# karltan0328/POPE

Hardware: AMD Instinct MI355X
Metric: image-pairs/s (DINOv2-S/14 extract+match, 640x480) (higher is better)
Workload: dtype f16x3 (fp32 operands split hi+lo into f16, 3 MFMAs per product, fp32 accumulate)

## Files before the change

### pope_amd/csrc/gemm_rowln.hip

```cpp
#include "gemm_core.h"
#include "gemm_routes.h"

namespace {

typedef _Float16 f16x4 __attribute__((ext_vector_type(4)));
typedef _Float16 f16x8 __attribute__((ext_vector_type(8)));
typedef __attribute__((ext_vector_type(4))) unsigned u32x4;
typedef __attribute__((ext_vector_type(2))) unsigned u32x2;

constexpr int RN = 384, RK = 32;
constexpr int ROWB = 64;
template <int RM_, int NWM_> struct RlGeo {
    static constexpr int RM = RM_, NWM = NWM_, NW = 4 * NWM, RTH = 64 * NW;
    static constexpr int NMI = RM / NWM / 16;
    static constexpr int STAGE_H = (RM + RN) * ROWB;
    static constexpr size_t STATS_OFF = size_t(2) * STAGE_H * sizeof(_Float16);
    static constexpr size_t CTAB_OFF = STATS_OFF + size_t(2) * 4 * RM * sizeof(float);
    static constexpr size_t PF_OFF = CTAB_OFF + size_t(4) * RN * sizeof(float);
    static constexpr size_t LDS_BYTES = PF_OFF + size_t(NW) * 256;
    static constexpr int EROWS = size_t(NW) * 16 * 100 * sizeof(float) <= size_t(STAGE_H) * sizeof(_Float16) ? 16 : 8;
    static constexpr int AROWS = RM / NW, WROWS = RN / NW;
    static constexpr int NPF = (RM * 12 + RTH - 1) / RTH;
    static_assert(size_t(NW) * EROWS * 100 * sizeof(float) <= size_t(STAGE_H) * sizeof(_Float16), "transposition buffers must fit a stage");
    static_assert(LDS_BYTES <= 160 * 1024, "LDS of a CU");
    static_assert(WROWS % 8 == 0 && AROWS % 8 == 0 && RM == NWM * NMI * 16, "eight rows per staging instruction");
};
typedef __attribute__((address_space(3))) void* lds_void_ptr;
constexpr float A_SCALE = K_PLANES_ACT_SCALE, W_SCALE = K_PLANES_W_SCALE;

__device__ __forceinline__ int pope_lane_id() {
    unsigned z = 0;
    asm volatile("" : "+s"(z));
    return int(__builtin_amdgcn_mbcnt_hi(~0u, __builtin_amdgcn_mbcnt_lo(~0u, z)));
}
__device__ __forceinline__ f32x4 mfma16(f16x8 a, f16x8 b, f32x4 c) {
    return __builtin_amdgcn_mfma_f32_16x16x32_f16(a, b, c, 0, 0, 0);
}
__device__ __forceinline__ float quad_sum(float v) {
    float a, b;
    pope_xor16_pair(v, a, b);
    pope_xor32_pair(a + b, a, b);
    return a + b;
}

#ifdef RL_STAMPS
__device__ unsigned long long g_rl_dbg[3][64];
#define RL_STAMP(slot)                                                                                             \
    do {                                                                                                           \
        if (LN && blockIdx.x == 0 && threadIdx.x == 0 && rl_si + (slot) < 64)        \
            g_rl_dbg[g.K == 384 ? 0 : (g.K == 1536 ? 1 : 2)][rl_si + (slot)] = wall_clock64();                     \
    } while (0)
#else
#define RL_STAMP(slot) do {} while (0)
#endif

__device__ __forceinline__ void rl_barrier() {
    __builtin_amdgcn_fence(__ATOMIC_RELEASE, "workgroup", "local");
    __builtin_amdgcn_s_barrier();
    __builtin_amdgcn_fence(__ATOMIC_ACQUIRE, "workgroup", "local");
}

enum { RL_LN_PLANES = 0, RL_LN_F32 = 1, RL_BIAS_PLANES = 2, RL_GELU_PLANES = 3 };

template <class G, int MODE, bool RES_TABLE>
__global__ __launch_bounds__(G::RTH) void gemm_rowln16_kernel(const GemmParams g, int n_tiles, int ncol) {
    constexpr bool LN = MODE == RL_LN_PLANES || MODE == RL_LN_F32, LN_PLANES = MODE == RL_LN_PLANES;
    constexpr int RM = G::RM, NMI = G::NMI, RTH = G::RTH, STAGE_H = G::STAGE_H, EROWS = G::EROWS, AROWS = G::AROWS, WROWS = G::WROWS;
    constexpr int WMR = 16 * NMI;
    constexpr int NIA = AROWS / 8, NIW = WROWS / 8;
    extern __shared__ __attribute__((aligned(16))) float smem[];
    _Float16* lds = reinterpret_cast<_Float16*>(smem);
    float* stats = reinterpret_cast<float*>(reinterpret_cast<char*>(smem) + G::STATS_OFF);
    float* ctab = reinterpret_cast<float*>(reinterpret_cast<char*>(smem) + G::CTAB_OFF);

    const int tid = threadIdx.x, lane = tid & 63;
    const int wave = __builtin_amdgcn_readfirstlane(tid >> 6);
    const int wm = wave >> 2, wn = wave & 3;
    const int nk = g.K / RK;
    const unsigned lda4 = unsigned(g.lda) * 4u, ldw4 = unsigned(g.ldw) * 4u;
    const __amdgpu_buffer_rsrc_t ra = __builtin_amdgcn_make_buffer_rsrc(const_cast<void*>(g.a_pl), 0, unsigned(g.M) * lda4, 0x00020000);
    const __amdgpu_buffer_rsrc_t rw = __builtin_amdgcn_make_buffer_rsrc(const_cast<void*>(g.w_pl), 0, unsigned(g.N) * ldw4, 0x00020000);
    auto row_tile = [&](int t) -> int { return LN ? t : t / ncol; };
    auto col_tile = [&](int t) -> int { return LN ? 0 : t - (t / ncol) * ncol; };

    const int grid = gridDim.x, full_rounds = n_tiles / grid;
    const int remapped = xcd_remap(blockIdx.x, grid);
    const int tail_cand = full_rounds * grid + int(blockIdx.x);
    const int tail_tile = tail_cand < n_tiles ? tail_cand : n_tiles;
    auto tile_of = [&](int ord) -> int {
        const int in_tail = pope_uniform_select(ord == full_rounds, tail_tile, n_tiles);
        return pope_uniform_select(ord < full_rounds, ord * grid + remapped, in_tail);
    };
    const int first = tile_of(0);
    if (first >= n_tiles) return;
    if (LN && tid < RN) {
        const float gm = g.gamma ? g.gamma[tid] : 1.0f;
        ctab[tid] = gm * (1.0f / (A_SCALE * W_SCALE));
        ctab[RN + tid] = (g.bias ? g.bias[tid] : 0.f) * gm;
        ctab[2 * RN + tid] = g.ln_w[tid];
        ctab[3 * RN + tid] = g.ln_b[tid];
    }

    const unsigned a8 = 8u * lda4, w8 = 8u * ldw4;
    auto dma = [&](int stage, int t, int kt_) {
        int ln_ = pope_lane_id();
        asm volatile("" : "+v"(ln_));
        const int r8 = ln_ >> 3, piece = (ln_ & 7) ^ r8;
        const int lt = t < n_tiles ? t : n_tiles - 1;
        _Float16* S_ = lds + stage * STAGE_H;
        const unsigned vt = unsigned(row_tile(lt) * RM + AROWS * wave + r8) * lda4 + unsigned(piece) * 16u;
        const unsigned ko = unsigned(kt_) * 128u + unsigned(col_tile(lt)) * unsigned(RN) * ldw4;
        const unsigned vw0 = unsigned(WROWS * wave + r8) * ldw4 + unsigned(piece) * 16u;
#pragma unroll
        for (int i = 0; i < NIA; ++i)
            __builtin_amdgcn_raw_ptr_buffer_load_lds(ra, (lds_void_ptr)(S_ + (AROWS * wave + 8 * i) * ROWB), 16, vt + i * a8, unsigned(kt_) * 128u, 0, LN ? 3 : 0);
#pragma unroll
        for (int i = 0; i < NIW; ++i)
            __builtin_amdgcn_raw_ptr_buffer_load_lds(rw, (lds_void_ptr)(S_ + (RM + WROWS * wave + 8 * i) * ROWB), 16, vw0, ko + i * w8, 0, 0);
    };
    f32x4 acc[NMI][6];
    auto zero_acc = [&]() {
#pragma unroll
        for (int mi = 0; mi < NMI; ++mi)
#pragma unroll
            for (int ni = 0; ni < 6; ++ni) acc[mi][ni] = f32x4{0.f, 0.f, 0.f, 0.f};
    };

    const __amdgpu_buffer_rsrc_t rx = __builtin_amdgcn_make_buffer_rsrc(g.C, 0, unsigned(g.M) * unsigned(RN) * 4u, 0x00020000);
    const __amdgpu_buffer_rsrc_t rln = __builtin_amdgcn_make_buffer_rsrc(LN_PLANES ? g.ln_planes : static_cast<void*>(g.ln_f32), 0,
                                                                         unsigned(g.M) * unsigned(RN) * 4u, 0x00020000);
    const __amdgpu_buffer_rsrc_t rres = __builtin_amdgcn_make_buffer_rsrc(
        const_cast<float*>(g.res), 0, unsigned(RES_TABLE ? g.res_mod : g.M) * unsigned(g.ldres) * 4u, 0x00020000);

    lds_void_ptr pf_pad = (lds_void_ptr)(reinterpret_cast<char*>(smem) + G::PF_OFF + wave * 256);
    auto prefetch_res = [&](int tile_, int j) {
        int t_ = wave * 64 + pope_lane_id();
        asm volatile("" : "+v"(t_));
        const unsigned L = unsigned(t_) + unsigned(RTH) * unsigned(j), row = L / 12u, pc = L - 12u * row;
        const unsigned off = RM * 12 % RTH == 0 || L < unsigned(RM * 12) ? (unsigned(tile_) * RM + row) * unsigned(RN) * 4u + pc * 128u : 0xFFFFFF00u;
        __builtin_amdgcn_raw_ptr_buffer_load_lds(rres, pf_pad, 4, off, 0, 0, 0);
    };

    int rl_si = 0;
    [[maybe_unused]] auto epilogue = [&](int tile, int free_stage) {
        const int m0 = tile * RM;
        float* wreg = reinterpret_cast<float*>(lds + free_stage * STAGE_H) + wave * (EROWS * 100);
        int elane = pope_lane_id();
        asm volatile("" : "+v"(elane));
        RL_STAMP(1);
        int l15 = elane & 15, q4 = elane >> 4;
        asm volatile("" : "+v"(l15), "+v"(q4));
        const int er = l15 & (EROWS - 1);
#pragma unroll
        for (int mi = 0; mi < NMI; ++mi)
#pragma unroll
            for (int ni = 0; ni < 6; ++ni) asm volatile("" : "+v"(acc[mi][ni]));
        const int col0 = wn * 96 + 4 * q4;
#pragma unroll
        for (int ni = 0; ni < 6; ++ni) {
            const f32x4 gam = *reinterpret_cast<const f32x4*>(ctab + col0 + 16 * ni);
            const f32x4 bia = *reinterpret_cast<const f32x4*>(ctab + RN + col0 + 16 * ni);
#pragma unroll
            for (int mi = 0; mi < NMI; ++mi) {
                const unsigned row = unsigned(m0 + wm * WMR + mi * 16 + l15);
                const unsigned rr = RES_TABLE ? row % unsigned(g.res_mod) : row;
                const f32x4 r = __builtin_bit_cast(f32x4, __builtin_amdgcn_raw_buffer_load_b128(
                                    rres, rr * unsigned(g.ldres) * 4u + unsigned(col0) * 4u, ni * 64, 0));
                acc[mi][ni] = r + acc[mi][ni] * gam + bia;
            }
#pragma unroll
            for (int mi = 0; mi < NMI; ++mi) asm volatile("" : "+v"(acc[mi][ni]));
            __builtin_amdgcn_sched_barrier(0);
        }
        __builtin_amdgcn_sched_barrier(0);
        RL_STAMP(2);
        const int rl = wm * WMR + l15;
#pragma unroll
        for (int mi = 0; mi < NMI; ++mi) {
            float s = 0.f;
#pragma unroll
            for (int ni = 0; ni < 6; ++ni) s += (acc[mi][ni][0] + acc[mi][ni][1]) + (acc[mi][ni][2] + acc[mi][ni][3]);
            s = quad_sum(s);
            if (q4 == 0) stats[wn * RM + rl + 16 * mi] = s;
        }
        rl_barrier();
        float mean[NMI], rstd[NMI];
#pragma unroll
        for (int mi = 0; mi < NMI; ++mi) {
            const float* p = stats + rl + 16 * mi;
            mean[mi] = ((p[0] + p[RM]) + (p[2 * RM] + p[3 * RM])) * (1.0f / float(RN));
        }
        __builtin_amdgcn_sched_barrier(0);
        RL_STAMP(3);
        auto store_lines = [&](const __amdgpu_buffer_rsrc_t& rdst, int row_base) {
            int el = elane;
            asm volatile("" : "+v"(el));
            const int epiece = el & 7;
#pragma unroll
            for (int t = 0; t < (EROWS * 3) / 8; ++t) {
                const int L = t * 8 + (el >> 3), row = (L * 43) >> 7, ln = L - 3 * row;
                const f32x4 v = *reinterpret_cast<const f32x4*>(&wreg[row * 100 + ln * 32 + epiece * 4]);
                const unsigned off = unsigned(row_base + row) * unsigned(RN) * 4u + unsigned(wn * 96 + ln * 32 + epiece * 4) * 4u;
                __builtin_amdgcn_raw_buffer_store_b128(__builtin_bit_cast(u32x4, v), rdst, off, 0, 0);
            }
        };
#pragma unroll
        for (int mi = 0; mi < NMI; ++mi) {
#pragma unroll
            for (int h = 0; h < 16 / EROWS; ++h) {
                if (EROWS == 16 || (l15 >> 3) == h) {
#pragma unroll
                    for (int ni = 0; ni < 6; ++ni) *reinterpret_cast<f32x4*>(&wreg[er * 100 + ni * 16 + 4 * q4]) = acc[mi][ni];
                }
                __builtin_amdgcn_wave_barrier();
                store_lines(rx, m0 + wm * WMR + mi * 16 + h * EROWS);
                __builtin_amdgcn_wave_barrier();
            }
        }
#pragma unroll
        for (int mi = 0; mi < NMI; ++mi) {
            float qs = 0.f;
#pragma unroll
            for (int ni = 0; ni < 6; ++ni) {
                const f32x4 d = acc[mi][ni] - mean[mi];
                acc[mi][ni] = d;
                qs += (d[0] * d[0] + d[1] * d[1]) + (d[2] * d[2] + d[3] * d[3]);
            }
            qs = quad_sum(qs);
            if (q4 == 0) stats[4 * RM + wn * RM + rl + 16 * mi] = qs;
        }
        rl_barrier();
#pragma unroll
        for (int mi = 0; mi < NMI; ++mi) {
            const float* p = stats + 4 * RM + rl + 16 * mi;
            const float var = ((p[0] + p[RM]) + (p[2 * RM] + p[3 * RM])) * (1.0f / float(RN));
            rstd[mi] = 1.0f / sqrtf(var + g.ln_eps);
        }
        __builtin_amdgcn_sched_barrier(0);
        RL_STAMP(4);
        const int live = g.M - (m0 + rl);
        float finite_probe = 0.f;
#pragma unroll
        for (int mi = 0; mi < NMI; ++mi) finite_probe += 16 * mi < live ? __builtin_fabsf(mean[mi]) + rstd[mi] : 0.f;
        f32x2 amax = {0.f, 0.f};
#pragma unroll
        for (int mi = 0; mi < NMI; ++mi) {
#pragma unroll
            for (int h = 0; h < 16 / EROWS; ++h) {
                if (EROWS == 16 || (l15 >> 3) == h) {
#pragma unroll
                    for (int ni = 0; ni < 6; ++ni) {
                        const f32x4 lw = *reinterpret_cast<const f32x4*>(ctab + 2 * RN + col0 + 16 * ni);
                        const f32x4 lb = *reinterpret_cast<const f32x4*>(ctab + 3 * RN + col0 + 16 * ni);
                        const f32x4 y = acc[mi][ni] * rstd[mi] * lw + lb;
                        if constexpr (LN_PLANES) {
                            const f32x4 ys = y * A_SCALE;
                            pope_amax4x2(amax, 16 * mi < live ? ys : f32x4{0.f, 0.f, 0.f, 0.f});
                            f16x4 hi, lo;
                            pope_split4(ys, hi, lo);
                            const int c = ni * 16 + 4 * q4;
                            _Float16* hp = reinterpret_cast<_Float16*>(wreg) + er * 200 + pope_planes_col(c);
                            *reinterpret_cast<f16x4*>(hp) = hi;
                            *reinterpret_cast<f16x4*>(hp + 32) = lo;
                        } else {
                            *reinterpret_cast<f32x4*>(&wreg[er * 100 + ni * 16 + 4 * q4]) = y;
                        }
                    }
                }
                __builtin_amdgcn_wave_barrier();
                store_lines(rln, m0 + wm * WMR + mi * 16 + h * EROWS);
                __builtin_amdgcn_wave_barrier();
            }
        }
        if constexpr (LN_PLANES)
            pope_range_flag(g.range_flag, POPE_RANGE_LAYERNORM,
                            !(__builtin_fmaxf(amax[0], amax[1]) < POPE_F16_OVERFLOW) ||
                                !(finite_probe < INFINITY));
        RL_STAMP(5);
    };

    const __amdgpu_buffer_rsrc_t rcp = __builtin_amdgcn_make_buffer_rsrc(LN ? static_cast<void*>(g.C) : g.c_pl, 0,
                                                                         unsigned(g.M) * unsigned(g.ldc) * 4u, 0x00020000);
    [[maybe_unused]] auto epilogue_planes = [&](int tile, int free_stage) {
        const int m0 = row_tile(tile) * RM, n0 = col_tile(tile) * RN;
        float* wreg = reinterpret_cast<float*>(lds + free_stage * STAGE_H) + wave * (EROWS * 100);
        int elane = pope_lane_id();
        asm volatile("" : "+v"(elane));
        int l15 = elane & 15, q4 = elane >> 4;
        asm volatile("" : "+v"(l15), "+v"(q4));
        const int er = l15 & (EROWS - 1);
#pragma unroll
        for (int mi = 0; mi < NMI; ++mi)
#pragma unroll
            for (int ni = 0; ni < 6; ++ni) asm volatile("" : "+v"(acc[mi][ni]));
        const int col0 = n0 + wn * 96 + 4 * q4;
        constexpr float inv = 1.0f / (A_SCALE * W_SCALE);
        f32x4 bias[6];
#pragma unroll
        for (int ni = 0; ni < 6; ++ni) bias[ni] = g.bias ? *reinterpret_cast<const f32x4*>(g.bias + col0 + 16 * ni) : f32x4{0.f, 0.f, 0.f, 0.f};
        f32x2 amax = {0.f, 0.f};
#pragma unroll
        for (int mi = 0; mi < NMI; ++mi) {
#pragma unroll
            for (int h = 0; h < 16 / EROWS; ++h) {
                if (EROWS == 16 || (l15 >> 3) == h) {
#pragma unroll
                    for (int ni = 0; ni < 6; ++ni) {
                        f32x4 v = acc[mi][ni] * inv + bias[ni];
                        if constexpr (MODE == RL_GELU_PLANES) {
                            const f32x2 g01 = pope_gelu_erf_pair(f32x2{v[0], v[1]}), g23 = pope_gelu_erf_pair(f32x2{v[2], v[3]});
                            v = f32x4{g01[0], g01[1], g23[0], g23[1]};
                        }
                        pope_amax4x2(amax, v);
                        f16x4 hi, lo;
                        pope_split4(v * A_SCALE, hi, lo);
                        const int c = ni * 16 + 4 * q4;
                        _Float16* hp = reinterpret_cast<_Float16*>(wreg) + er * 200 + pope_planes_col(c);
                        *reinterpret_cast<f16x4*>(hp) = hi;
                        *reinterpret_cast<f16x4*>(hp + 32) = lo;
                    }
                }
                __builtin_amdgcn_wave_barrier();
                {
                    int el = elane;
                    asm volatile("" : "+v"(el));
                    const int epiece = el & 7;
                    const int row_base = m0 + wm * WMR + mi * 16 + h * EROWS;
#pragma unroll
                    for (int t = 0; t < (EROWS * 3) / 8; ++t) {
                        const int L = t * 8 + (el >> 3), row = (L * 43) >> 7, ln = L - 3 * row;
                        const f32x4 v = *reinterpret_cast<const f32x4*>(&wreg[row * 100 + ln * 32 + epiece * 4]);
                        const unsigned off = unsigned(row_base + row) * unsigned(g.ldc) * 4u + unsigned(n0 + wn * 96 + ln * 32 + epiece * 4) * 4u;
                        __builtin_amdgcn_raw_buffer_store_b128(__builtin_bit_cast(u32x4, v), rcp, off, 0, 2);
                    }
                }
                __builtin_amdgcn_wave_barrier();
            }
        }
        pope_range_flag(g.range_flag, g.range_bit, !(__builtin_fmaxf(amax[0], amax[1]) * A_SCALE < POPE_F16_OVERFLOW));
    };

    dma(0, first, 0);
    zero_acc();
    int tile = first, kt = 0, ord = 0, next_tile = tile_of(1);
    RL_STAMP(0);

    for (int s = 0; tile < n_tiles; ++s) {
        if (!LN || kt != 0 || ord == 0) __builtin_amdgcn_s_waitcnt(0x0f70);
        rl_barrier();
        const bool seam = kt + 1 == nk;
        dma((s + 1) & 1, seam ? next_tile : tile, seam ? 0 : kt + 1);
        const _Float16* S = lds + (s & 1) * STAGE_H;
        int fl_ = pope_lane_id();
        asm volatile("" : "+v"(fl_));
        const int fl15 = fl_ & 15, fq4 = fl_ >> 4;
        const int sw_hi = 8 * (fq4 ^ (fl15 & 7)), sw_lo = 8 * ((4 + fq4) ^ (fl15 & 7));
        const int a_row = (wm * WMR + fl15) * ROWB, w_row = (RM + wn * 96 + fl15) * ROWB;
        f16x8 ah[NMI], al[NMI], wl[2], wh[2];
        wl[0] = *reinterpret_cast<const f16x8*>(S + w_row + sw_lo);
#pragma unroll
        for (int t = 0; t < NMI; ++t) ah[t] = *reinterpret_cast<const f16x8*>(S + a_row + t * 16 * ROWB + sw_hi);
        wh[0] = *reinterpret_cast<const f16x8*>(S + w_row + sw_hi);
#pragma unroll
        for (int t = 0; t < NMI; ++t) al[t] = *reinterpret_cast<const f16x8*>(S + a_row + t * 16 * ROWB + sw_lo);
        __builtin_amdgcn_sched_barrier(0);
#pragma unroll
        for (int ni = 0; ni < 6; ++ni) {
            const int cur = ni & 1, nxt = cur ^ 1;
            if (ni + 1 < 6) {
                wl[nxt] = *reinterpret_cast<const f16x8*>(S + w_row + (ni + 1) * 16 * ROWB + sw_lo);
                wh[nxt] = *reinterpret_cast<const f16x8*>(S + w_row + (ni + 1) * 16 * ROWB + sw_hi);
            }
            if constexpr (LN && !RES_TABLE)
                if (ni == 2 && g.rl_prefetch && kt >= nk - 1 - G::NPF && kt < nk - 1 && nk > G::NPF) prefetch_res(tile, kt - (nk - 1 - G::NPF));
#pragma unroll
            for (int mi = 0; mi < NMI; ++mi) acc[mi][ni] = mfma16(wl[cur], ah[mi], acc[mi][ni]);
#pragma unroll
            for (int mi = 0; mi < NMI; ++mi) acc[mi][ni] = mfma16(wh[cur], al[mi], acc[mi][ni]);
#pragma unroll
            for (int mi = 0; mi < NMI; ++mi) acc[mi][ni] = mfma16(wh[cur], ah[mi], acc[mi][ni]);
            __builtin_amdgcn_sched_barrier(0);
        }
        if (++kt == nk) {
            rl_barrier();
            if constexpr (LN) epilogue(tile, s & 1);
            else epilogue_planes(tile, s & 1);
            zero_acc();
            kt = 0;
            tile = next_tile;
            next_tile = tile_of(++ord + 1);
            rl_si += 8;
            RL_STAMP(0);
        }
    }
    __builtin_amdgcn_s_waitcnt(0x0f70);
}

template <class G, int MODE, bool RES_TABLE>
int launch_rowln_geo(const GemmParams& g, hipStream_t stream) {
    const int ncol = (g.N + RN - 1) / RN;
    const int tiles = ((g.M + G::RM - 1) / G::RM) * ncol, cus = pope_cu_count();
    return pope_launch_lds<gemm_rowln16_kernel<G, MODE, RES_TABLE>>(dim3(tiles < cus ? tiles : cus), dim3(G::RTH), G::LDS_BYTES, stream,
                                                                    g, tiles, ncol);
}

template <int MODE, bool RES_TABLE>
int launch_rowln(const GemmParams& g, hipStream_t stream) {
    const long long cus = pope_cu_count(), ncol = (g.N + RN - 1) / RN;
    const long long r128 = (((g.M + 127) / 128) * ncol + cus - 1) / cus * 128, r192 = (((g.M + 191) / 192) * ncol + cus - 1) / cus * 192;
    return r192 <= r128 ? launch_rowln_geo<RlGeo<192, 2>, MODE, RES_TABLE>(g, stream)
                        : launch_rowln_geo<RlGeo<128, 2>, MODE, RES_TABLE>(g, stream);
}

}

#ifdef RL_STAMPS
extern "C" int pope_lab_rowln_stamps(unsigned long long* host192) {
    return hipMemcpyFromSymbol(host192, HIP_SYMBOL(g_rl_dbg), sizeof(unsigned long long) * 192) == hipSuccess ? 0 : -1;
}
#endif

bool pope_gemm_rowln_supported(const GemmParams& g) {
    return g.N == RN && g.ldc == RN && g.K >= 2 * RK && (g.K % RK) == 0 && g.lda == g.K && g.ldw == g.K && g.ldres == RN &&
           size_t(g.M + 192) * g.lda * 4 < (size_t(1) << 32) && size_t(g.M + 192) * RN * 4 < (size_t(1) << 32) - 512;
}

bool pope_gemm_rowln_args_ok(const GemmParams& g) {
    if (!g.a_pl || !g.w_pl || !g.C || !g.res || !g.ln_w || !g.ln_b || (!g.ln_planes) == (!g.ln_f32) || g.M <= 0) return false;
    if (!pope_gemm_rowln_supported(g)) return false;
    return g.res_mod >= 0 && (g.res_mod > 0 || g.gamma);
}

int pope_launch_gemm_rowln(const GemmParams& g_in, hipStream_t stream) {
    GemmParams g = g_in;
    g.rl_prefetch = 1;
    if (!pope_gemm_rowln_args_ok(g)) return POPE_ERR_ARG;
    if (g.res_mod > 0) return g.ln_planes ? launch_rowln<RL_LN_PLANES, true>(g, stream) : launch_rowln<RL_LN_F32, true>(g, stream);
    return g.ln_planes ? launch_rowln<RL_LN_PLANES, false>(g, stream) : launch_rowln<RL_LN_F32, false>(g, stream);
}

bool pope_stream384_supported(const GemmParams& g) {
    if (g.plain || !g.a_pl || !g.w_pl || !g.c_pl || g.conv_cch > 0 || g.nbatch > 1) return false;
    if (g.epilogue != EPI_BIAS && g.epilogue != EPI_BIAS_GELU) return false;
    if (g.N % RN || g.K < 2 * RK || (g.K % RK) || g.lda != g.K || g.ldw != g.K || g.ldc != g.N) return false;
    if (size_t(g.M + 192) * g.lda * 4 >= (size_t(1) << 32) || size_t(g.N) * g.ldw * 4 >= (size_t(1) << 32) ||
        size_t(g.M + 192) * g.ldc * 4 >= (size_t(1) << 32) - 512)
        return false;
    return size_t((g.M + 191) / 192) * (g.N / RN) >= size_t(4) * pope_cu_count();
}

int pope_launch_stream384(const GemmParams& g, hipStream_t stream) {
    return g.epilogue == EPI_BIAS_GELU ? launch_rowln_geo<RlGeo<192, 2>, RL_GELU_PLANES, false>(g, stream)
                                       : launch_rowln_geo<RlGeo<192, 2>, RL_BIAS_PLANES, false>(g, stream);
}
```

Baseline: 1472.

## Stagger SIMD-partner waves by deferring last MFMA blocks across the stage barrier

Waves 4-7, which share SIMDs with waves 0-3, now run only the first 6-LAG column blocks of each K-step. They keep the remaining weight fragments in registers and issue those MFMAs at the start of the next step, after the barrier. This puts partner waves out of phase so one wave's MFMA bursts overlap the other's LDS reads and barrier waits, instead of both contending at once. The cost is extra VGPRs for the deferred fragments, an extra waitcnt, role dispatch branching, and a flush before the epilogue. The timing-stamp instrumentation is also extended to record per-wave-group data.

```diff
diff --git a/pope_amd/csrc/gemm_rowln.hip b/pope_amd/csrc/gemm_rowln.hip
--- a/pope_amd/csrc/gemm_rowln.hip
+++ b/pope_amd/csrc/gemm_rowln.hip
@@ -1,3 +1,5 @@
+#include <type_traits>
+
 #include "gemm_core.h"
 #include "gemm_routes.h"
 
@@ -43,15 +45,25 @@
     return a + b;
 }
 
+#ifndef RL_LAG
+#define RL_LAG 3
+#endif
+#ifndef RL_LAG_STAGE_BEHIND
+#define RL_LAG_STAGE_BEHIND 1
+#endif
+
 #ifdef RL_STAMPS
-__device__ unsigned long long g_rl_dbg[3][64];
-#define RL_STAMP(slot)                                                                                             \
+__device__ unsigned long long g_rl_dbg[2][3][64];
+#define RL_STAMP_IF(cond, slot)                                                                                    \
     do {                                                                                                           \
-        if (LN && blockIdx.x == 0 && threadIdx.x == 0 && rl_si + (slot) < 64)        \
-            g_rl_dbg[g.K == 384 ? 0 : (g.K == 1536 ? 1 : 2)][rl_si + (slot)] = wall_clock64();                     \
+        if (LN && blockIdx.x == 0 && (threadIdx.x & 255) == 0 && (cond) && rl_si + (slot) < 64)    \
+            g_rl_dbg[threadIdx.x >> 8][g.K == 384 ? 0 : (g.K == 1536 ? 1 : 2)][rl_si + (slot)] = wall_clock64();   \
     } while (0)
+#define RL_STAMP(slot) RL_STAMP_IF(true, slot)
+#define RL_STAMP_K(slot) RL_STAMP_IF(kt == 1, slot)
 #else
 #define RL_STAMP(slot) do {} while (0)
+#define RL_STAMP_K(slot) do {} while (0)
 #endif
 
 __device__ __forceinline__ void rl_barrier() {
@@ -345,18 +357,43 @@
     int tile = first, kt = 0, ord = 0, next_tile = tile_of(1);
     RL_STAMP(0);
 
-    for (int s = 0; tile < n_tiles; ++s) {
-        if (!LN || kt != 0 || ord == 0) __builtin_amdgcn_s_waitcnt(0x0f70);
-        rl_barrier();
+    constexpr int LAG = RL_LAG;
+    static_assert(LAG >= 0 && LAG <= 3 && G::NW == 8, "waves 4 - 7 are the SIMD partners of waves 0 - 3");
+    [[maybe_unused]] const bool late = LAG > 0 && wave >= 4;
+    enum { ROLE_IN_PHASE = 0, ROLE_LATE_FIRST = 1, ROLE_LATE = 2 };
+    f16x8 ah[NMI], al[NMI];
+    [[maybe_unused]] f16x8 dwl[LAG > 0 ? LAG : 1], dwh[LAG > 0 ? LAG : 1];
+    auto mfma_block = [&](int ni, const f16x8& l, const f16x8& h, [[maybe_unused]] bool first_of_step) {
+#pragma unroll
+        for (int mi = 0; mi < NMI; ++mi) {
+            acc[mi][ni] = mfma16(l, ah[mi], acc[mi][ni]);
+            if (first_of_step && mi == 0) RL_STAMP_K(7);
+        }
+#pragma unroll
+        for (int mi = 0; mi < NMI; ++mi) acc[mi][ni] = mfma16(h, al[mi], acc[mi][ni]);
+#pragma unroll
+        for (int mi = 0; mi < NMI; ++mi) acc[mi][ni] = mfma16(h, ah[mi], acc[mi][ni]);
+    };
+    [[maybe_unused]] auto deferred_blocks = [&]() {
+#pragma unroll
+        for (int j = 0; j < LAG; ++j) mfma_block(6 - LAG + j, dwl[j], dwh[j], j == 0);
+    };
+    auto kstep = [&](auto role_c, int s_, const _Float16* S) {
+        constexpr int ROLE = decltype(role_c)::value;
+        constexpr int NOW = ROLE == ROLE_IN_PHASE ? 6 : 6 - LAG;
         const bool seam = kt + 1 == nk;
-        dma((s + 1) & 1, seam ? next_tile : tile, seam ? 0 : kt + 1);
-        const _Float16* S = lds + (s & 1) * STAGE_H;
+        if constexpr (ROLE == ROLE_LATE && RL_LAG_STAGE_BEHIND) {
+            deferred_blocks();
+            __builtin_amdgcn_sched_barrier(0);
+        }
+        dma((s_ + 1) & 1, seam ? next_tile : tile, seam ? 0 : kt + 1);
+        if constexpr (ROLE == ROLE_LATE && !RL_LAG_STAGE_BEHIND) deferred_blocks();
         int fl_ = pope_lane_id();
         asm volatile("" : "+v"(fl_));
         const int fl15 = fl_ & 15, fq4 = fl_ >> 4;
         const int sw_hi = 8 * (fq4 ^ (fl15 & 7)), sw_lo = 8 * ((4 + fq4) ^ (fl15 & 7));
         const int a_row = (wm * WMR + fl15) * ROWB, w_row = (RM + wn * 96 + fl15) * ROWB;
-        f16x8 ah[NMI], al[NMI], wl[2], wh[2];
+        f16x8 wl[2], wh[2];
         wl[0] = *reinterpret_cast<const f16x8*>(S + w_row + sw_lo);
 #pragma unroll
         for (int t = 0; t < NMI; ++t) ah[t] = *reinterpret_cast<const f16x8*>(S + a_row + t * 16 * ROWB + sw_hi);
@@ -365,24 +402,50 @@
         for (int t = 0; t < NMI; ++t) al[t] = *reinterpret_cast<const f16x8*>(S + a_row + t * 16 * ROWB + sw_lo);
         __builtin_amdgcn_sched_barrier(0);
 #pragma unroll
-        for (int ni = 0; ni < 6; ++ni) {
+        for (int ni = 0; ni < NOW; ++ni) {
             const int cur = ni & 1, nxt = cur ^ 1;
-            if (ni + 1 < 6) {
+            if (ni + 1 < NOW) {
                 wl[nxt] = *reinterpret_cast<const f16x8*>(S + w_row + (ni + 1) * 16 * ROWB + sw_lo);
                 wh[nxt] = *reinterpret_cast<const f16x8*>(S + w_row + (ni + 1) * 16 * ROWB + sw_hi);
+            } else if constexpr (ROLE != ROLE_IN_PHASE) {
+#pragma unroll
+                for (int j = 0; j < LAG; ++j) {
+                    dwl[j] = *reinterpret_cast<const f16x8*>(S + w_row + (NOW + j) * 16 * ROWB + sw_lo);
+                    dwh[j] = *reinterpret_cast<const f16x8*>(S + w_row + (NOW + j) * 16 * ROWB + sw_hi);
+                }
             }
             if constexpr (LN && !RES_TABLE)
                 if (ni == 2 && g.rl_prefetch && kt >= nk - 1 - G::NPF && kt < nk - 1 && nk > G::NPF) prefetch_res(tile, kt - (nk - 1 - G::NPF));
-#pragma unroll
-            for (int mi = 0; mi < NMI; ++mi) acc[mi][ni] = mfma16(wl[cur], ah[mi], acc[mi][ni]);
-#pragma unroll
-            for (int mi = 0; mi < NMI; ++mi) acc[mi][ni] = mfma16(wh[cur], al[mi], acc[mi][ni]);
-#pragma unroll
-            for (int mi = 0; mi < NMI; ++mi) acc[mi][ni] = mfma16(wh[cur], ah[mi], acc[mi][ni]);
+            mfma_block(ni, wl[cur], wh[cur], ROLE != ROLE_LATE && ni == 0);
             __builtin_amdgcn_sched_barrier(0);
+        }
+    };
+
+    for (int s = 0; tile < n_tiles; ++s) {
+        if (!LN || kt != 0 || ord == 0) __builtin_amdgcn_s_waitcnt(0x0f70);
+        if constexpr (LAG > 0) __builtin_amdgcn_s_waitcnt(0xc07f);
+        rl_barrier();
+        RL_STAMP_K(6);
+        const _Float16* S = lds + (s & 1) * STAGE_H;
+        if constexpr (LAG > 0) {
+            int role = pope_uniform_select(late, pope_uniform_select(kt == 0, int(ROLE_LATE_FIRST), int(ROLE_LATE)), int(ROLE_IN_PHASE));
+            if (role == ROLE_IN_PHASE) kstep(std::integral_constant<int, ROLE_IN_PHASE>{}, s, S);
+            asm volatile("" : "+s"(role));
+            if (role == ROLE_LATE_FIRST) kstep(std::integral_constant<int, ROLE_LATE_FIRST>{}, s, S);
+            asm volatile("" : "+s"(role));
+            if (role == ROLE_LATE) kstep(std::integral_constant<int, ROLE_LATE>{}, s, S);
+        } else {
+            kstep(std::integral_constant<int, ROLE_IN_PHASE>{}, s, S);
         }
         if (++kt == nk) {
             rl_barrier();
+            if constexpr (LAG > 0) {
+                if (late) deferred_blocks();
+#pragma unroll
+                for (int t = 0; t < NMI; ++t) ah[t] = __builtin_nondeterministic_value(ah[t]), al[t] = __builtin_nondeterministic_value(al[t]);
+#pragma unroll
+                for (int j = 0; j < LAG; ++j) dwl[j] = __builtin_nondeterministic_value(dwl[j]), dwh[j] = __builtin_nondeterministic_value(dwh[j]);
+            }
             if constexpr (LN) epilogue(tile, s & 1);
             else epilogue_planes(tile, s & 1);
             zero_acc();
@@ -415,8 +478,8 @@
 }
 
 #ifdef RL_STAMPS
-extern "C" int pope_lab_rowln_stamps(unsigned long long* host192) {
-    return hipMemcpyFromSymbol(host192, HIP_SYMBOL(g_rl_dbg), sizeof(unsigned long long) * 192) == hipSuccess ? 0 : -1;
+extern "C" int pope_lab_rowln_stamps(unsigned long long* host384) {
+    return hipMemcpyFromSymbol(host384, HIP_SYMBOL(g_rl_dbg), sizeof(unsigned long long) * 384) == hipSuccess ? 0 : -1;
 }
 #endif
 
```

Result: faster. 1496, median of 6 (+1.6%).
